# CognitiveAISystems/pogema

Measured on AMD Instinct MI355X. Metric: agent-steps/sec (whole node), 64-agent 64x64 grid, batch=8192 envs, higher is better.
Workload: dtype u32

## Files before the change

include/pogema_amd.h:

```cpp
#ifndef POGEMA_AMD_H
#define POGEMA_AMD_H

#include <stddef.h>
#include <stdint.h>

#ifdef __cplusplus
extern "C" {
#endif

#define PGX_ABI_VERSION 6

#define PGX_OK 0
#define PGX_E_INVALID (-1)
#define PGX_E_HIP (-2)
#define PGX_E_NOMEM (-3)
#define PGX_E_STATE (-4)
#define PGX_E_PLACEMENT (-5)

#define PGX_COLLISION_PRIORITY 0
#define PGX_COLLISION_BLOCK_BOTH 1
#define PGX_COLLISION_SOFT 2

#define PGX_ON_TARGET_FINISH 0
#define PGX_ON_TARGET_RESTART 1
// ... 71 lines not shown
int pgx_set_map_pool(pgx_env* env, const uint8_t* maps, int32_t num_maps, int32_t* capacity_out, void* stream);
int pgx_reset_pool(pgx_env* env, uint64_t seed, const uint8_t* env_mask, int32_t max_retries, void* stream);
int pgx_regenerate_pool(pgx_env* env, const uint8_t* env_mask, uint64_t seed, int32_t max_retries, void* obs,
                        void* stream);
int pgx_get_map_index(pgx_env* env, int32_t* map_index, void* stream);

int pgx_get_map(pgx_env* env, uint8_t* obstacles, void* stream);

int pgx_step(pgx_env* env, const void* actions, int action_dtype, void* obs, float* rewards,
             uint8_t* terminated, uint8_t* truncated, uint8_t* is_active, void* stream);

int pgx_step_held(pgx_env* env, const void* actions, int action_dtype, void* obs, uint8_t* held, int32_t refresh,
                  float* rewards, uint8_t* terminated, uint8_t* truncated, uint8_t* is_active, void* stream);
int pgx_held_available(const pgx_env* env);

int pgx_xcd_shares(pgx_env* env, int32_t* shares);
int pgx_xcd_tune(pgx_env* env, void* obs, void* obs_alt, int32_t rounds, float* us_equal, float* us_tuned, void* stream);

typedef struct pgx_geometry {
    int32_t lanes_per_env;
    int32_t waves;
    int32_t envs_per_wave;
    int32_t multi_wave;
    int32_t p16;
    int32_t stagger;
    int32_t store_policy;
    int32_t state_stores;
    int32_t grid;
    int32_t lds_bytes;
    int32_t for_rollout;
// ... 193 lines not shown
```

pogema_amd/_lib.py:

```python
from __future__ import annotations

import ctypes as C
import os

_HERE = os.path.dirname(os.path.abspath(__file__))
LIB_PATH = os.environ.get("PGX_LIB") or os.path.join(_HERE, "libpogema_amd.so")

PGX_ABI_VERSION = 6

COLLISION_SYSTEMS = {"priority": 0, "block_both": 1, "soft": 2}
ON_TARGET = {"finish": 0, "restart": 1, "nothing": 2}
ACTION_DTYPES = {"int8": 0, "int32": 1, "int64": 2}
SOFT_VERTEX_RULES = {"lowest_index": 0, "all_stay": 1}
SOFT_OCCUPANCY = {"index_order": 0, "exact": 1}
COOP_REWARDS = {"all_solved": 0, "per_agent": 1}
BAD_ACTIONS = {"noop": 0, "flag": 1}
LIFELONG_RNGS = {"build": 0, "numpy": 1}
def _obs_dtypes():
    import torch
    return {torch.float32: 0, torch.uint8: 1, torch.bfloat16: 2, torch.float16: 3}


def obs_elem_bytes(dtype) -> int:
    import torch
# ... 58 lines not shown
          "GREEDY0": TOKEN_GREEDY0, "PAD": TOKEN_PAD, "NUM_TOKENS": NUM_TOKENS, "HISTORY": TOKEN_HISTORY,
          "SLOT_LEN": TOKEN_SLOT_LEN, "MAX_SLOTS": MAX_TOKEN_SLOTS, "MAX_LENGTH": MAX_TOKEN_LENGTH}


EXPORTED_SYMBOLS = (
    "pgx_abi_version", "pgx_last_error", "pgx_create", "pgx_check_config", "pgx_destroy", "pgx_obs_elems", "pgx_agent_elems",
    "pgx_reset_from_state", "pgx_reset_random", "pgx_regenerate", "pgx_regenerate_failures", "pgx_get_map", "pgx_step", "pgx_step_held", "pgx_held_available", "pgx_observe", "pgx_set_metrics_buffers", "pgx_get_state", "pgx_generate", "pgx_place_agents",
    "pgx_snapshot_bytes", "pgx_save_snapshot", "pgx_load_snapshot", "pgx_time_observe", "pgx_bad_action_count",
    "pgx_buffers_create", "pgx_buffers_ptr", "pgx_buffers_get_info", "pgx_buffers_destroy", "pgx_set_targets",
    "pgx_np_streams", "pgx_np_streams_host", "pgx_np_generate", "pgx_np_generate_host", "pgx_rollout", "pgx_buffers_stride", "pgx_buffers_drop", "pgx_xcd_shares", "pgx_xcd_tune", "pgx_buffers_create_at", "pgx_time_observe_pair", "pgx_buffers_va_reserved", "pgx_get_geometry",
    "pgx_expert_actions", "pgx_set_map_pool", "pgx_reset_pool", "pgx_regenerate_pool", "pgx_get_map_index",
    "pgx_cost_to_go", "pgx_cost_to_go_bytes", "pgx_cost_to_go_builds", "pgx_visible_agents", "pgx_pibt_actions",
    "pgx_goal_directions", "pgx_shield_actions", "pgx_pibt_plan", "pgx_move_outcomes",
    "pgx_policy_input", "pgx_copy_envs", "pgx_global_state", "pgx_global_state_check",
    "pgx_agent_tokens", "pgx_agent_tokens_length", "pgx_goal_paths", "pgx_pibt_swap_actions",
    "pgx_agent_forecasts", "pgx_blocking",
)


class PgxError(RuntimeError):
    def __init__(self, code: int, message: str):
        super().__init__(f"pogema_amd engine error {code}: {message}")
        self.code = code


class PgxBuffersInfo(C.Structure):
    _fields_ = [("bytes", C.c_int64), ("count", C.c_int32), ("spread", C.c_int32), ("candidates", C.c_int32),
                ("reserved0", C.c_int32), ("same_zone_us", C.c_float), ("final_us", C.c_float), ("spacer_gib", C.c_double),
                ("buffer_gbs", C.c_float), ("reserved1", C.c_float)]


# ... 138 lines not shown
    lib.pgx_bad_action_count.argtypes = [vp, vp]
    lib.pgx_bad_action_count.restype = i64
    lib.pgx_time_observe.argtypes = [vp, vp, i32, C.POINTER(C.c_float), vp]
    lib.pgx_time_observe.restype = C.c_int
    lib.pgx_time_observe_pair.argtypes = [vp, vp, vp, i32, C.POINTER(C.c_float), vp]
    lib.pgx_time_observe_pair.restype = C.c_int
    lib.pgx_snapshot_bytes.argtypes = [vp]
    lib.pgx_snapshot_bytes.restype = i64
    lib.pgx_save_snapshot.argtypes = [vp, vp, vp]
    lib.pgx_load_snapshot.argtypes = [vp, vp, vp]
    lib.pgx_save_snapshot.restype = lib.pgx_load_snapshot.restype = C.c_int
    lib.pgx_step.argtypes = [vp, vp, C.c_int, vp, vp, vp, vp, vp, vp]
    lib.pgx_step_held.argtypes = [vp, vp, C.c_int, vp, vp, i32, vp, vp, vp, vp, vp]
    lib.pgx_held_available.argtypes = [vp]
    lib.pgx_step_held.restype = lib.pgx_held_available.restype = C.c_int
    lib.pgx_observe.argtypes = [vp, vp, vp]
    lib.pgx_set_metrics_buffers.argtypes = [vp, vp, vp]
    lib.pgx_get_state.argtypes = [vp, vp, vp, vp, vp, vp, vp]
    lib.pgx_generate.argtypes = [i32, i32, i32, i32, f32, u64, i64, i32, i32, vp, vp, vp]
    lib.pgx_place_agents.argtypes = [i32, i32, i32, i32, u64, i64, i32, i32, vp, i32, vp, vp]
    for name in ("pgx_create", "pgx_destroy", "pgx_reset_from_state", "pgx_reset_random", "pgx_regenerate", "pgx_get_map",
                 "pgx_step", "pgx_observe", "pgx_set_metrics_buffers", "pgx_set_metrics_buffers",
                 "pgx_get_state", "pgx_generate", "pgx_place_agents"):
        getattr(lib, name).restype = C.c_int
    if lib.pgx_abi_version() != PGX_ABI_VERSION:
        raise ImportError(f"{LIB_PATH}: ABI version {lib.pgx_abi_version()} != expected {PGX_ABI_VERSION}; rebuild")
    _lib = lib
    return lib


# ... 5 lines not shown
```

pogema_amd/buffers.py:

```python
from __future__ import annotations

import atexit
import collections
import contextlib
import ctypes as C
import os
import threading

import numpy as np
import torch

from . import _lib

_TYPESTR = {torch.float32: "<f4", torch.uint8: "|u1", torch.float16: "<f2", torch.bfloat16: "<f2"}


class _Owner:

    def __init__(self, lib, handle):
        self._lib, self._handle = lib, handle

    def __del__(self):
        try:
            if self._handle is not None and self._handle.value:
# ... 322 lines not shown
        dev = obs_tensors[0].device
        n = batch * agents
        self._sets = []
        for obs in obs_tensors:
            block = torch.empty(n * 7 + 16, dtype=torch.uint8, device=dev)
            members = (obs, block[:4 * n].view(torch.float32).view(batch, agents),
                       block[4 * n:5 * n].view(torch.bool).view(batch, agents),
                       block[5 * n:6 * n].view(torch.bool).view(batch, agents),
                       block[6 * n:7 * n].view(torch.bool).view(batch, agents))
            storages = (obs.untyped_storage(), block.untyped_storage())
            self._sets.append((members, storages, tuple(st._cdata for st in storages)))
        del obs, block, members, storages
        self._idle = [tuple(self._count(c) for c in cdata) for _, _, cdata in self._sets]
        self._held = [torch.full((batch, agents), 255, dtype=torch.uint8, device=dev) for _ in self._sets]
        self._vouched = [None] * len(self._sets)
        self._next = 0
        self.taken = 0
        self.misses = 0

    def __len__(self):
        return len(self._sets)

    def obs_pointers(self):
        return [members[0].data_ptr() for members, _, _ in self._sets]

    def _is_idle(self, i: int) -> bool:
        cdata, idle = self._sets[i][2], self._idle[i]
        return self._count(cdata[0]) == idle[0] and self._count(cdata[1]) == idle[1]

    def free_sets(self) -> int:
        return sum(self._is_idle(i) for i in range(len(self._sets)))

    def retire(self):
        idle = [i for i in range(len(self._sets)) if self._is_idle(i)]
        out = [self._sets[i][0][0] for i in idle if self._sets[i][0][0].data_ptr() in self._zone_ptrs]
        for i in reversed(idle):
            del self._sets[i]
            del self._idle[i]
            del self._held[i]
            del self._vouched[i]
        self._next = 0
        return out

    def _take_index(self):
        n = len(self._sets)
        for k in range(n):
            i = (self._next + k) % n
            if self._is_idle(i):
                self._next = (i + 1) % n
                self.taken += 1
                return i
        self.misses += 1
        return None

    def _hand_out(self, i: int, with_obs: bool):
# ... 14 lines not shown
        if with_obs:
            self._vouched[i] = None
        return self._hand_out(i, with_obs)

    def take_for_step(self, with_obs: bool = True):
        i = self._take_index()
        if i is None:
            return None
        trusted = False
        if with_obs:
            v = self._vouched[i]
            trusted = v is not None and self._version(self._sets[i][0][0]) == v
            self._vouched[i] = None
        return self._hand_out(i, with_obs), self._held[i], trusted, i

    def vouch(self, i: int):
        self._vouched[i] = self._version(self._sets[i][0][0])
```

pogema_amd/csrc/pgx_api.cpp:

```cpp
#include "../../include/pogema_amd.h"

#include <hip/hip_runtime.h>

#include <algorithm>
#include <cstdarg>
#include <cstdio>
#include <cstdlib>
#include <cstring>
#include <new>
#include <string>
#include <vector>

#include "pgx_internal.h"

namespace {
thread_local std::string g_err;
}

namespace pgx {
int fail_msg(int code, const char* fmt, ...) {
    char buf[512];
    va_list ap;
    va_start(ap, fmt);
    vsnprintf(buf, sizeof buf, fmt, ap);
// ... 350 lines not shown
        alloc(e->tcount, BA * sizeof(uint32_t));
        if (cfg->lifelong_rng == PGX_LIFELONG_RNG_NUMPY) {
            alloc(e->np_state, BA * sizeof(pgx::NpGen));
            alloc(e->np_state0, BA * sizeof(pgx::NpGen));
        }
    }
    if (err != hipSuccess) return fail_msg(alloc_code(err), "hipMalloc failed: %s", hipGetErrorString(err));
    err = hipMemset(e->regen_fail, 0, sizeof(uint32_t));
    if (err == hipSuccess) err = hipMemset(e->bad_count, 0, sizeof(uint32_t));
    if (err == hipSuccess && e->np_state0)
        err = pgx::launch_init_np_lifelong(e->np_state0, cfg->seed, cfg->env_index_base, cfg->batch, A, nullptr);
    if (err == hipSuccess && e->np_state0) err = hipStreamSynchronize(nullptr);
    if (err == hipSuccess) err = pgx::prepare_step(e->geo, e->geo_roll);
    if (err == hipSuccess && pgx::held_available(e->geo, A, e->W, obs_elem_bytes(cfg->obs_dtype)))
        err = pgx::prepare_step_held(e->geo, A, e->W);
    if (err != hipSuccess)
        return fail_msg(PGX_E_HIP, "cannot configure the step kernel (%zu bytes of LDS): %s", e->geo.lds_bytes,
                        hipGetErrorString(err));
    if (const char* spec = getenv("PGX_XCD_WEIGHTS")) {
        float f[8], sum = 0.f;
        if (sscanf(spec, "%f,%f,%f,%f,%f,%f,%f,%f", &f[0], &f[1], &f[2], &f[3], &f[4], &f[5], &f[6], &f[7]) == 8) {
            for (float q : f) sum += q > 0.f ? q : 0.f;
            if (sum > 0.f)
                for (int x = 0; x < 8; ++x) e->xcd_w[x] = (f[x] > 0.f ? f[x] : 0.f) / sum;
        }
    }
    apply_xcd_shares(e);
    err = pgx::prepare_expert(cfg->height, cfg->width);
    if (err != hipSuccess) return fail_msg(PGX_E_HIP, "cannot configure the expert kernel: %s", hipGetErrorString(err));
    if (e->flags & 4u) {
// ... 537 lines not shown
        return pgx_step(e, actions, action_dtype, obs, rewards, terminated, truncated, is_active, stream);
    if (!actions || !rewards || !terminated || !truncated) return fail_msg(PGX_E_INVALID, "pgx_step_held: null argument");
    if (const int rc = check_action_dtype("pgx_step_held", action_dtype)) return rc;
    DeviceGuard guard;
    if (const int rc = enter(guard, e, "pgx_step_held", true)) return rc;
    pgx::StepParams p = step_params(e, e->geo);
    p.mode = pgx::MODE_STEP;
    p.action_dtype = action_dtype;
    p.actions = actions;
    p.obs = static_cast<float*>(obs);
    p.rewards = rewards;
    p.terminated = terminated;
    p.truncated = truncated;
    p.act_out = is_active;
    PGX_HIP(pgx::launch_step_held(p, e->geo, held, refresh != 0, (hipStream_t)stream));
    return PGX_OK;
}

int pgx_rollout(pgx_env* e, int32_t steps, const pgx_rollout_io* io, void* stream) {
    if (!e || !io || !io->rewards || !io->terminated || !io->truncated)
        return fail_msg(PGX_E_INVALID, "pgx_rollout: null argument");
    if (io->policy_step0 < 0 || io->policy_step0 > ((int64_t)1 << 40))
        return fail_msg(PGX_E_INVALID, "pgx_rollout: policy_step0 outside 0..2^40");
    if (steps < 1) return fail_msg(PGX_E_INVALID, "pgx_rollout: steps must be >= 1, got %d", steps);
    if (const int rc = check_action_dtype("pgx_rollout", io->action_dtype)) return rc;
    if (io->obs && io->obs_slots < 1) return fail_msg(PGX_E_INVALID, "pgx_rollout: obs given but obs_slots = %d", io->obs_slots);
    DeviceGuard guard;
    if (const int rc = enter(guard, e, "pgx_rollout", true)) return rc;
    pgx::StepParams p = step_params(e, e->geo_roll);
    p.mode = pgx::MODE_STEP;
// ... 716 lines not shown
```

pogema_amd/csrc/pgx_internal.h:

```cpp
#pragma once
#include <hip/hip_runtime.h>
#include <stddef.h>
#include <stdint.h>

namespace pgx {

int fail_msg(int code, const char* fmt, ...);

#define PGX_HIP(call)                                                                                                      \
    do {                                                                                                                   \
        const hipError_t e__ = (call);                                                                                     \
        if (e__ != hipSuccess)                                                                                             \
            return pgx::fail_msg(PGX_E_HIP, "%s failed: %s (%s:%d)", #call, hipGetErrorString(e__), __FILE__, __LINE__); \
    } while (0)

struct DeviceGuard {
    int prev = -1;
    bool changed = false;
    hipError_t err = hipSuccess;
    DeviceGuard() = default;
    explicit DeviceGuard(int dev) { (void)select(dev); }
    DeviceGuard(const DeviceGuard&) = delete;
    DeviceGuard& operator=(const DeviceGuard&) = delete;
    hipError_t select(int dev) {
// ... 100 lines not shown
    const void* actions;
    float* obs;
    float* rewards;
    uint8_t* terminated;
    uint8_t* truncated;
    uint8_t* act_out;
    const uint8_t* only;
    unsigned long long* dbg;
};

struct HeldParams {
    uint8_t* held;
    int32_t refresh;
    int32_t lds_word;
    int32_t words;
};

struct RolloutParams {
    int32_t steps;
    int32_t obs_slots;
    int32_t resident_bitmap;
    int32_t reserved0;
    int64_t actions_stride;
    int64_t agents_stride;
    int64_t envs_stride;
    int64_t obs_stride;
    uint64_t policy_seed;
    int64_t policy_step0;
    int8_t* actions_out;
};
// ... 10 lines not shown
    bool big;
    bool pc;
    bool resident_bitmap;
    size_t lds_bytes;
    int grid;
    int32_t xcd_n[8], xcd_base[8];
};
StepGeometry step_geometry(int batch, int A, int bmw, int W, bool allow_p16, int epw_override, int obs_elem_bytes,
                           int waves_override, bool for_rollout = false);
hipError_t prepare_step(const StepGeometry& g, const StepGeometry& roll);
hipError_t raise_lds_limit(const void* fn, size_t lds_bytes);
hipError_t launch_step(const StepParams& p, const StepGeometry& g, hipStream_t stream);
bool held_available(const StepGeometry& g, int A, int W, int obs_elem_bytes);
hipError_t prepare_step_held(const StepGeometry& g, int A, int W);
hipError_t launch_step_held(const StepParams& p, const StepGeometry& g, uint8_t* held, bool refresh, hipStream_t stream);
int xcd_partition(int blocks, const float w[8], int32_t n[8], int32_t base[8]);
hipError_t launch_rollout(const StepParams& p, const RolloutParams& rp, const StepGeometry& g, hipStream_t stream);

hipError_t launch_pack_obstacles(const uint8_t* obstacles, const uint8_t* only, uint32_t* bm, int batch, int H, int Wd,
                                 int r, int wpr, int bmw, const OutsideParams& outside, hipStream_t stream);

struct ResetParams {
    int32_t env_begin, env_count;
    int32_t H, Wd, A, r, wpr, bmw;
    int32_t lifelong;
    int32_t given_state;
    int32_t max_retries;
    uint32_t thr;
    uint64_t gen_seed;
    int64_t env_index_base;
// ... 230 lines not shown
```

pogema_amd/csrc/pgx_kernels.hip:

```cpp
#include <hip/hip_runtime.h>
#include <stdint.h>
#include <stdlib.h>

#include <array>
#include <type_traits>
#include <map>
#include <mutex>
#include <string>
#include <vector>
#include <utility>

#include "pgx_internal.h"
#include "pgx_nprng.h"

namespace pgx {

__device__ __forceinline__ uint32_t lifelong_draw(uint64_t seed, uint64_t env_index, uint32_t agent,
                                                  uint32_t counter, uint32_t n) {
    uint64_t h = gen_sm64(seed);
    h = gen_sm64(h ^ env_index);
    h = gen_sm64(h ^ (((uint64_t)agent << 32) | counter));
    return (uint32_t)(((h >> 32) * (uint64_t)n) >> 32);
}

// ... 317 lines not shown
        }
    }
}

enum { MISC_FLAGS = 0, MISC_ARRIVED = 16, MISC_UNSOLVED = 17, MISC_OFFGOAL = 18, MISC_WORDS = 32 };

struct Carry {
    uint32_t pos = 0u, tgt = 1u;
    uint32_t ablk = 0u, anext = 0u;
    int elapsed = 0;
    int4 macc = {0, 0, 0, 0};
    bool active = false;
};
__device__ __forceinline__ uint32_t pack_action4(int a) { return (uint32_t)a <= 4u ? (uint32_t)a : 15u; }

template <int G, bool MW, bool P16, bool ROLL, bool BIG, bool PC, bool HELD, typename P, typename R, typename H = int>
__device__ __forceinline__ void step_body(P& p, R& rp, const int t, const int slot, Carry& c, [[maybe_unused]] const H& hp = H{}) {
    static_assert(!MW || G == 64, "multi-wave environments use full waves");
    static_assert(!HELD || (P16 && !ROLL && !BIG && !PC), "the held stream exists for the packed-row single-step kernels");
    static_assert(!BIG || MW, "the large-map layout runs one environment per workgroup");
    static_assert(!PC || (ROLL && !MW && P16), "the resolver / streamer pair exists for single-wave rollouts with packed rows");
    extern __shared__ __attribute__((aligned(16))) uint32_t smem[];

    const int tid = PC ? (int)(threadIdx.x & 63u) : (int)threadIdx.x;
    [[maybe_unused]] const int role = PC ? (int)(threadIdx.x >> 6) : 0;
    bool do_resolve = true;
    [[maybe_unused]] bool do_stream = true;
    if constexpr (PC) {
        do_resolve = role == 0 && t < rp.steps;
        do_stream = role == 1 && t > 0;
        if (!do_resolve && !do_stream) return;
// ... 43 lines not shown
    const int env_l = MW ? 0 : (lane / G);
    const int gbase = MW ? 0 : (lane & ~(G - 1));
    const int alane = MW ? lane : (lane & (G - 1));
    const int agent = MW ? tid : alane;
    const bool env_ok = env_l < nenv;
    const int env = env0 + env_l;
    const bool valid = env_ok && agent < A;
    const size_t gi = (size_t)env * A + agent;

    uint32_t pos = 0u, tgt = 1u;
    bool active = false;
    bool ghost_in = false;
    int act = 0, elapsed = 0;
    int4 macc = make_int4(0, 0, 0, 0);
    bool env_leader;
    [[maybe_unused]] int araw[8];
    [[maybe_unused]] bool fetch_block = false;
    if constexpr (ROLL) {
      env_leader = env_ok && agent == 0 && p.mode == MODE_STEP;
      if (do_resolve) {
        auto load_action = [&](size_t ai) -> int {
            if (p.action_dtype == 0) return ((const int8_t*)p.actions)[ai];
            if (p.action_dtype == 1) return ((const int32_t*)p.actions)[ai];
            return (int)((const int64_t*)p.actions)[ai];
        };
        const bool given = p.actions != nullptr;
        const int steps = rp.steps;
        const size_t stride = (size_t)rp.agents_stride;
        if (t == 0) {
            if (valid) {
// ... 37 lines not shown
    if (valid) {
        pos = p.pos[gi];
        tgt = p.tgt[gi];
        const uint32_t ab = p.active[gi];
        active = (ab & ACTIVE_BIT) != 0;
        ghost_in = (ab & ACTIVE_GHOST) != 0;
        if (p.mode == MODE_STEP) {
            if (p.action_dtype == 0) act = ((const int8_t*)p.actions)[gi];
            else if (p.action_dtype == 1) act = ((const int32_t*)p.actions)[gi];
            else act = (int)((const int64_t*)p.actions)[gi];
        }
    }
    if (env_ok && p.mode == MODE_STEP) elapsed = p.elapsed[env];
    env_leader = env_ok && agent == 0 && p.mode == MODE_STEP;
    if (env_leader) macc = p.macc[env];
    }

    if (do_resolve) {
        const uint32_t* g = p.obst + (size_t)env0 * bmw;
        const int n = nenv * bmw;
        const int stagger = (ROLL && t > 0) ? 0 : p.stagger;
        bool stage = true;
        if constexpr (ROLL) stage = t == 0 || !rp.resident_bitmap;
        if constexpr (BIG) stage = false;
        if (!stage) {
#pragma unroll 4
            for (int i = tid; i < n; i += NT) s_occ[i] = 0u;
        } else if (!MW && stagger > 0 && n <= 16 * 64) {
            uint32_t bmr[16];
#pragma unroll
// ... 3 lines not shown
            if (slot & 1u)
                for (int k = 0; k < stagger; ++k) __builtin_amdgcn_s_sleep(127);
#pragma unroll
            for (int k = 0; k < 16; ++k)
                if (tid + 64 * k < n) {
                    s_obst[tid + 64 * k] = bmr[k];
                    s_occ[tid + 64 * k] = 0u;
                }
        } else
#pragma unroll 4
        for (int i = tid; i < n; i += NT) {
            s_obst[i] = g[i];
            s_occ[i] = 0u;
        }
        if (MW && tid < MISC_WORDS) s_misc[tid] = 0u;
    }
    lds_sync<MW>();
    const bool dbg2 = dbg && (p.flags & 64u);
    if (dbg2 && tid == 0) p.dbg[(size_t)blk * 4 + 1] = wall_clock64();

    bool ghost = p.mode != MODE_STEP && ghost_in;
    struct StateOut {
        float rew = 0.0f;
        uint8_t term = 0;
        bool trunc = false, finished = false, do_reset = false, act = false;
        int n_arrived = 0;
    } so;
    int when_stores = p.mode == MODE_STEP ? p.state_stores : 0;
    if constexpr (PC) when_stores = 0;
    const bool late_stores = when_stores != 0;
// ... 230 lines not shown
            uint32_t b = 0u;
#pragma unroll
            for (int k = 0; k < 8; ++k) b |= pack_action4(araw[k]) << (4 * k);
            c.anext = b;
        }
      }
    }
    if (dbg && tid == 0) p.dbg[(size_t)blk * 4 + (dbg2 ? 3 : 1)] = wall_clock64();
    if (!p.obs) {
        if (late_stores) emit_state(pos, tgt, active, elapsed, macc, so);
        return;
    }
    if constexpr (PC) {
        if (!do_stream) return;
    }
    if constexpr (HELD) {
        for (int i = tid; i < hp.words; i += NT) smem[hp.lds_word + i] = 0u;
    }
    lds_sync<MW>();
    if (when_stores == 1) emit_state(pos, tgt, active, elapsed, macc, so);
    int out_slot = slot;
    if constexpr (PC) out_slot = slot == 0 ? rp.obs_slots - 1 : slot - 1;
    float* const obs_out = ROLL ? reinterpret_cast<float*>(reinterpret_cast<char*>(p.obs) + (size_t)out_slot * (size_t)rp.obs_stride) : p.obs;

    if constexpr (P16) {
        const int W_rt = W, r_rt = r;
        uint32_t* rows_base = smem;
        if constexpr (ROLL) rows_base = rp.resident_bitmap ? s_occ : smem;
        if constexpr (PC) rows_base = s_obst + epw * bmw + 2 * (epw * bmw + 2 * AS);
        auto p16_phases = [&](auto wt_tag) {
        constexpr int WT = decltype(wt_tag)::value;
        const int W = WT ? WT : W_rt;
        const int r = WT ? (WT - 1) / 2 : r_rt;
        const uint32_t wmask = (1u << W) - 1u;
        constexpr int RW = WT ? (WT + 1) / 2 : 8;
        [[maybe_unused]] uint32_t held_was = 255u;
        if constexpr (HELD) {
            if (tid < nag && !hp.refresh) held_was = hp.held[(size_t)env0 * A + tid];
        }
        uint32_t rp[3][RW];
#pragma unroll
        for (int t = 0; t < 3; ++t) {
#pragma unroll
            for (int m = 0; m < RW; ++m) rp[t][m] = 0u;
            const int item = tid + t * NT;
            if (item < nag * 3) {
                const int la = item / 3;
                const int c = item - la * 3;
                const int el = MW ? 0 : (p.a_magic ? (int)__umulhi((uint32_t)la, p.a_magic) : la);
                const uint32_t cell = s_apos[la];
                const int x = (int)(cell >> 16), y = (int)(cell & 0xFFFFu);
                if (c < 2) {
// ... 36 lines not shown
                            asm volatile("" ::: "memory");
                        }
                    }
                } else {
                    const uint32_t tc = s_atgt[la];
                    int dx = x - (int)(tc >> 16), dy = y - (int)(tc & 0xFFFFu);
                    dx = max(-r, min(r, dx));
                    dy = max(-r, min(r, dy));
                    const int hit = r - dx;
                    const uint32_t val = (1u << (r - dy)) << (16 * (hit & 1));
#pragma unroll
                    for (int m = 0; m < RW; ++m) rp[t][m] = (m == (hit >> 1)) ? val : 0u;
                }
            }
        }
        if constexpr (HELD) {
            if (tid < nag) {
                const int la = tid;
                const uint32_t cell = s_apos[la], tc = s_atgt[la];
                const int dx = max(-r, min(r, (int)(cell >> 16) - (int)(tc >> 16)));
                const int dy = max(-r, min(r, (int)(cell & 0xFFFFu) - (int)(tc & 0xFFFFu)));
                const uint32_t now = (uint32_t)((r - dx) * W + (r - dy));
                hp.held[(size_t)env0 * A + la] = (uint8_t)now;
                if (held_was < (uint32_t)(W * W)) {
                    constexpr int UL = PGX_HELD_UNIT_LOG2;
                    const uintptr_t slice = reinterpret_cast<uintptr_t>(obs_out + (size_t)env0 * A * 3 * W * W);
                    const uintptr_t plane = slice + (size_t)(la * 3 + 2) * (size_t)(W * W) * 4;
                    const uintptr_t ub = slice >> UL;
                    const int u1 = (int)(((plane + (size_t)(W * W) * 4) >> UL) - ub);
                    const int uw = (int)(((plane + held_was * 4) >> UL) - ub), un = (int)(((plane + now * 4) >> UL) - ub);
                    for (int u = (int)(((plane + ((1u << UL) - 1u)) >> UL) - ub); u < u1; ++u)
// ... 2 lines not shown
            }
        }
        lds_sync<MW>();
        uint16_t* rows16 = reinterpret_cast<uint16_t*>(rows_base);
#pragma unroll
        for (int t = 0; t < 3; ++t) {
            const int item = tid + t * NT;
            if (item < nag * 3) {
#pragma unroll
                for (int wy = 0; wy < (WT ? WT : 16); ++wy)
                    if (WT || wy < W) rows16[item * W + wy] = (uint16_t)(rp[t][wy >> 1] >> (16 * (wy & 1)));
            }
        }
        if (tid < 4) rows16[nag * 3 * W + tid] = 0;
        lds_sync<MW>();

        const int n = nag * 3 * W * W;
        const size_t base = (size_t)env0 * A * 3 * W * W;
        if constexpr (WT == 0) {
        if (p.obs_one && W >= 7) {
            uint16_t* o = reinterpret_cast<uint16_t*>(obs_out) + base;
            const int head = min(n, (int)((8 - (base & 7)) & 7));
            const int nvec = (n - head) >> 3;
            const int tail0 = head + (nvec << 3);
            if (tid < 16) {
                const int e = (tid < 8) ? tid : tail0 + (tid - 8);
                if ((tid < 8) ? (tid < head) : (e < n)) {
                    const int row = (int)__umulhi((uint32_t)e, p.w_magic);
                    o[e] = (uint16_t)((((uint32_t)rows16[row] >> (e - row * W)) & 1u) * p.obs_one);
                }
// ... 164 lines not shown
        if (p.store_policy == 0) stream32(std::integral_constant<uint32_t, 0u>{});
        else if (p.store_policy == 1) stream32(std::integral_constant<uint32_t, 1u>{});
        else stream32(std::integral_constant<uint32_t, 2u>{});
        if (when_stores == 2) emit_state(pos, tgt, active, elapsed, macc, so);
        if (dbg && !dbg2 && tid == 0) {
            __builtin_amdgcn_s_waitcnt(0);
            p.dbg[(size_t)blk * 4 + 3] = wall_clock64();
        }
    }
}

template <int G, bool MW, bool P16, bool BIG = false>
__global__ __launch_bounds__(MW ? 1024 : 64, MW ? 1 : 8) void step_kernel(const StepParams p) {
    const RolloutParams none{};
    Carry unused;
    step_body<G, MW, P16, false, BIG, false, false>(p, none, 0, 0, unused);
}

template <int G, bool MW>
__global__ __launch_bounds__(MW ? 1024 : 64, MW ? 1 : 8) void step_held(const StepParams p, const HeldParams hp) {
    const RolloutParams none{};
    Carry unused;
    step_body<G, MW, true, false, false, false, true>(p, none, 0, 0, unused, hp);
}

#ifndef PGX_ROLL_OCC
#define PGX_ROLL_OCC 4
#endif
template <int G, bool MW, bool P16, bool BIG = false, bool PC = false>
__global__ __launch_bounds__(MW ? 1024 : (PC ? 128 : 64), MW ? 1 : PGX_ROLL_OCC) void rollout_kernel(const StepParams p0, const RolloutParams rp0) {
    typedef const __attribute__((address_space(4))) char KC;
    typedef const __attribute__((address_space(4))) StepParams KP;
    typedef const __attribute__((address_space(4))) RolloutParams KR;
    static_assert(alignof(StepParams) == 8 && alignof(RolloutParams) == 8, "kernarg layout of rollout_kernel");
    constexpr size_t rp_offset = (sizeof(StepParams) + alignof(RolloutParams) - 1) / alignof(RolloutParams) * alignof(RolloutParams);
    const int steps = rp0.steps, slots = rp0.obs_slots;
    int slot = 0;
    Carry c;
// ... 333 lines not shown
    return g.lds_bytes + (size_t)held_words(slice) * 4 <= 160 * 1024;
}

hipError_t prepare_step_held(const StepGeometry& g, int A, int W) {
    const size_t slice = (size_t)g.epw * A * 3 * W * W * 4;
    return raise_lds_limit(held_fn_for(g), g.lds_bytes + (size_t)held_words(slice) * 4);
}

hipError_t launch_step_held(const StepParams& p, const StepGeometry& g, uint8_t* held, bool refresh, hipStream_t stream) {
    const void* fn = held_fn_for(g);
    if (!fn) return hipErrorInvalidValue;
    StepParams args = p;
    HeldParams h;
    const int W = 2 * p.r + 1;
    h.held = held;
    h.refresh = refresh ? 1 : 0;
    h.lds_word = (int32_t)(g.lds_bytes / 4);
    h.words = held_words((size_t)g.epw * p.num_agents * 3 * W * W * 4);
    void* kargs[] = {&args, &h};
    return hipLaunchKernel(fn, dim3(g.grid), dim3(64 * g.waves), kargs, g.lds_bytes + (size_t)h.words * 4, stream);
}

hipError_t launch_step(const StepParams& p, const StepGeometry& g, hipStream_t stream) {
    const void* fn = step_fn_for(g);
    if (!fn) return hipErrorInvalidValue;
    StepParams args = p;
    void* kargs[] = {&args};
    return hipLaunchKernel(fn, dim3(g.grid), dim3(64 * g.waves), kargs, g.lds_bytes, stream);
}


hipError_t launch_pack_obstacles(const uint8_t* obstacles, const uint8_t* only, uint32_t* bm, int batch, int H, int Wd,
                                 int r, int wpr, int bmw, const OutsideParams& outside, hipStream_t stream) {
// ... 52 lines not shown
```

pogema_amd/vec_env.py:

```python
from __future__ import annotations

import ctypes as C
import os
import warnings
from typing import Optional

import numpy as np
import torch

from . import _lib
from .grid_config import GridConfig
from .placement import PlacementMixin, choose_buffers
from .queries import QueryMixin
from .semantics import Semantics


def _as_device_index(device) -> int:
    dev = torch.device(device)
    if dev.type != "cuda":
        raise ValueError(f"VecPogema runs on a HIP device only, got {device!r}")
    return dev.index if dev.index is not None else torch.cuda.current_device()


def parse_map_pool(maps) -> torch.Tensor:
# ... 167 lines not shown
            outside_density=float(gc.density), soft_vertex_rule=_lib.SOFT_VERTEX_RULES[self.semantics.soft_vertex],
            coop_reward=_lib.COOP_REWARDS[self.semantics.coop_reward],
            bad_action=_lib.BAD_ACTIONS[self.semantics.bad_action],
            lifelong_rng=_lib.LIFELONG_RNGS[self.semantics.lifelong_rng],
            soft_occupancy=_lib.SOFT_OCCUPANCY[self.semantics.soft_occupancy], abi_version=_lib.PGX_ABI_VERSION)
        self._handle = C.c_void_p()
        rc = self._lib.pgx_check_config(C.byref(cfg))
        if rc != 0:
            raise ValueError(f"this GridConfig does not fit the engine: {self._lib.pgx_last_error().decode()} (README.md, Limits)")
        _lib.check(self._lib.pgx_create(C.byref(cfg), self.device_index, C.byref(self._handle)))
        if held_zeros is None and os.environ.get("PGX_HELD_ZEROS") in ("0", "1"):
            held_zeros = os.environ["PGX_HELD_ZEROS"] == "1"
        self._held_on = ((self._held_pays() if held_zeros is None else bool(held_zeros)) and self.recycle
                         and self.obs_dtype == torch.float32 and not self.regenerate
                         and bool(self._lib.pgx_held_available(self._handle)))
        self._held_steps = 0
        self._held_refreshes = 0
        self._bufs = None
        self._buf_i = 0
        self._shared = None
        self._reset_seed = None
        self._initial = None
        self._pool = None
        self.metrics = torch.zeros((self.batch, len(_lib.METRIC_NAMES)), dtype=torch.float32, device=self.device)
        self.episode_done = torch.zeros((self.batch,), dtype=torch.bool, device=self.device)
        _lib.check(self._lib.pgx_set_metrics_buffers(self._handle, self.metrics.data_ptr(), self.episode_done.data_ptr()))
        if pool is not None:
            self.set_map_pool(pool)

    def close(self, release: bool = False):
# ... 317 lines not shown
        self.placement = dict(placement or {}, adopted=True)
        if self.placement_probe and self.batch >= 2048 and self._has_state():
            self.placement.update(self.tune_xcd_shares(tensors[0], tensors[-1] if len(tensors) > 1 else None))
        return self.placement

    def _has_state(self):
        return self._initial is not None

    HELD_MIN_BYTES = 128 << 20

    def _held_pays(self) -> bool:
        return int(np.prod(self.obs_shape)) * 4 >= self.HELD_MIN_BYTES

    @property
    def held_zeros(self) -> dict:
        return {"enabled": bool(self._held_on), "steps": self._held_steps, "refreshes": self._held_refreshes}

    def _outputs(self, with_obs: bool = True):
        if self.recycle:
            return self._recycled(with_obs)
        if not self.reuse_buffers:
            return self._alloc_outputs(with_obs)
        if self._bufs is None:
            if torch.cuda.is_current_stream_capturing():
                raise RuntimeError("reuse_buffers: the output buffers are picked by a timed zone walk that synchronises "
                                   "the device -- call warm_buffers() (or one un-captured step) before capturing")
            self.warm_buffers()
        self._buf_i = 0 if self.single_buffer else self._buf_i ^ 1
        return self._bufs[self._buf_i]

    def observe(self, out: Optional[torch.Tensor] = None) -> torch.Tensor:
# ... 34 lines not shown
            if tuple(t.shape) != tuple(shape) or not ok_dtype or not t.is_contiguous() or t.device != self.device:
                raise ValueError(f"out[{name}] must be a contiguous {dtype} tensor of shape {tuple(shape)} on {self.device}")
        return out

    def step(self, actions, compute_obs: bool = True, out=None):
        actions = self._prepare_actions(actions)
        if out is not None:
            obs, rewards, terminated, truncated, is_active = self._check_out(out)
            if compute_obs and obs is None:
                raise ValueError("out[obs] is None but compute_obs=True")
        else:
            held = self._held_outputs(compute_obs) if self._held_on else None
            if held is not None:
                (obs, rewards, terminated, truncated, is_active), record, trusted, index = held
                if compute_obs:
                    _lib.check(self._lib.pgx_step_held(
                        self._handle, actions.data_ptr(), self._ACTION_CODE[actions.dtype], obs.data_ptr(), record.data_ptr(),
                        0 if trusted else 1, rewards.data_ptr(), terminated.data_ptr(), truncated.data_ptr(),
                        is_active.data_ptr(), self._stream()))
                    self._recycler.vouch(index)
                    self._held_steps += 1
                    self._held_refreshes += 0 if trusted else 1
                    infos = {"is_active": is_active, "episode_done": self.episode_done, "metrics": self.metrics}
                    if self.semantics.bad_action == "flag":
                        self._raise_on_bad_actions()
                    return self._wrap_obs(obs), rewards, terminated, truncated, infos
            elif self._held_on and self._recycler and not torch.cuda.is_current_stream_capturing():
                obs, rewards, terminated, truncated, is_active = self._alloc_outputs(compute_obs)
            else:
                obs, rewards, terminated, truncated, is_active = self._outputs(compute_obs)
        _lib.check(self._lib.pgx_step(
# ... 178 lines not shown
```

Baseline: 5.344 billion.

## Add line-granular held-zero record to skip rewriting all-zero observation units

Adds a new held-stream step kernel variant that records, per 128-byte unit of each env slice's observation output, whether the unit was all zeros on the previous write into a recycled buffer. The kernel ORs packed row bits per unit, ballots the zero flags into a per-block bitmask kept in LDS and global memory, and uses it to skip stores of units that are already zero in the reused buffer. The aim is to cut global write bandwidth for float32 observations, replacing the per-agent target-based held rule. It costs extra LDS, a ballot pass and a record buffer per recycled set, and is picked by default only for large observations when the multi-wave helper layout does not apply.

```diff
diff --git a/include/pogema_amd.h b/include/pogema_amd.h
--- a/include/pogema_amd.h
+++ b/include/pogema_amd.h
@@ -109,6 +109,10 @@
                   float* rewards, uint8_t* terminated, uint8_t* truncated, uint8_t* is_active, void* stream);
 int pgx_held_available(const pgx_env* env);
 
+int pgx_step_held_lines(pgx_env* env, const void* actions, int action_dtype, void* obs, uint32_t* lines, int32_t refresh,
+                        float* rewards, uint8_t* terminated, uint8_t* truncated, uint8_t* is_active, void* stream);
+int64_t pgx_held_lines_words(const pgx_env* env);
+
 int pgx_xcd_shares(pgx_env* env, int32_t* shares);
 int pgx_xcd_tune(pgx_env* env, void* obs, void* obs_alt, int32_t rounds, float* us_equal, float* us_tuned, void* stream);
 
diff --git a/pogema_amd/_lib.py b/pogema_amd/_lib.py
--- a/pogema_amd/_lib.py
+++ b/pogema_amd/_lib.py
@@ -96,7 +96,7 @@
     "pgx_goal_directions", "pgx_shield_actions", "pgx_pibt_plan", "pgx_move_outcomes",
     "pgx_policy_input", "pgx_copy_envs", "pgx_global_state", "pgx_global_state_check",
     "pgx_agent_tokens", "pgx_agent_tokens_length", "pgx_goal_paths", "pgx_pibt_swap_actions",
-    "pgx_agent_forecasts", "pgx_blocking",
+    "pgx_agent_forecasts", "pgx_blocking", "pgx_step_held_lines", "pgx_held_lines_words",
 )
 
 
@@ -265,6 +265,10 @@
     lib.pgx_step_held.argtypes = [vp, vp, C.c_int, vp, vp, i32, vp, vp, vp, vp, vp]
     lib.pgx_held_available.argtypes = [vp]
     lib.pgx_step_held.restype = lib.pgx_held_available.restype = C.c_int
+    lib.pgx_step_held_lines.argtypes = [vp, vp, C.c_int, vp, vp, i32, vp, vp, vp, vp, vp]
+    lib.pgx_step_held_lines.restype = C.c_int
+    lib.pgx_held_lines_words.argtypes = [vp]
+    lib.pgx_held_lines_words.restype = i64
     lib.pgx_observe.argtypes = [vp, vp, vp]
     lib.pgx_set_metrics_buffers.argtypes = [vp, vp, vp]
     lib.pgx_get_state.argtypes = [vp, vp, vp, vp, vp, vp, vp]
diff --git a/pogema_amd/buffers.py b/pogema_amd/buffers.py
--- a/pogema_amd/buffers.py
+++ b/pogema_amd/buffers.py
@@ -360,6 +360,7 @@
         self._idle = [tuple(self._count(c) for c in cdata) for _, _, cdata in self._sets]
         self._held = [torch.full((batch, agents), 255, dtype=torch.uint8, device=dev) for _ in self._sets]
         self._vouched = [None] * len(self._sets)
+        self._lines = [None] * len(self._sets)
         self._next = 0
         self.taken = 0
         self.misses = 0
@@ -385,6 +386,7 @@
             del self._idle[i]
             del self._held[i]
             del self._vouched[i]
+            del self._lines[i]
         self._next = 0
         return out
 
@@ -429,5 +431,11 @@
             self._vouched[i] = None
         return self._hand_out(i, with_obs), self._held[i], trusted, i
 
+    def line_record(self, i: int, words: int):
+        rec = self._lines[i]
+        if rec is None or rec.numel() != words:
+            rec = self._lines[i] = torch.zeros(words, dtype=torch.int32, device=self._sets[i][0][0].device)
+        return rec
+
     def vouch(self, i: int):
         self._vouched[i] = self._version(self._sets[i][0][0])
diff --git a/pogema_amd/csrc/pgx_api.cpp b/pogema_amd/csrc/pgx_api.cpp
--- a/pogema_amd/csrc/pgx_api.cpp
+++ b/pogema_amd/csrc/pgx_api.cpp
@@ -388,6 +388,8 @@
     if (err == hipSuccess) err = pgx::prepare_step(e->geo, e->geo_roll);
     if (err == hipSuccess && pgx::held_available(e->geo, A, e->W, obs_elem_bytes(cfg->obs_dtype)))
         err = pgx::prepare_step_held(e->geo, A, e->W);
+    if (err == hipSuccess && pgx::held_lines_words(e->geo, cfg->batch, A, e->W, obs_elem_bytes(cfg->obs_dtype)))
+        err = pgx::prepare_step_held_lines(e->geo, A, e->W);
     if (err != hipSuccess)
         return fail_msg(PGX_E_HIP, "cannot configure the step kernel (%zu bytes of LDS): %s", e->geo.lds_bytes,
                         hipGetErrorString(err));
@@ -955,6 +957,32 @@
     p.truncated = truncated;
     p.act_out = is_active;
     PGX_HIP(pgx::launch_step_held(p, e->geo, held, refresh != 0, (hipStream_t)stream));
+    return PGX_OK;
+}
+
+int64_t pgx_held_lines_words(const pgx_env* e) {
+    if (!e) return 0;
+    return pgx::held_lines_words(e->geo, e->cfg.batch, e->cfg.num_agents, e->W, obs_elem_bytes(e->cfg.obs_dtype));
+}
+
+int pgx_step_held_lines(pgx_env* e, const void* actions, int action_dtype, void* obs, uint32_t* lines, int32_t refresh,
+                        float* rewards, uint8_t* terminated, uint8_t* truncated, uint8_t* is_active, void* stream) {
+    if (!e || !obs || !lines || !pgx_held_lines_words(e))
+        return pgx_step(e, actions, action_dtype, obs, rewards, terminated, truncated, is_active, stream);
+    if (!actions || !rewards || !terminated || !truncated) return fail_msg(PGX_E_INVALID, "pgx_step_held_lines: null argument");
+    if (const int rc = check_action_dtype("pgx_step_held_lines", action_dtype)) return rc;
+    DeviceGuard guard;
+    if (const int rc = enter(guard, e, "pgx_step_held_lines", true)) return rc;
+    pgx::StepParams p = step_params(e, e->geo);
+    p.mode = pgx::MODE_STEP;
+    p.action_dtype = action_dtype;
+    p.actions = actions;
+    p.obs = static_cast<float*>(obs);
+    p.rewards = rewards;
+    p.terminated = terminated;
+    p.truncated = truncated;
+    p.act_out = is_active;
+    PGX_HIP(pgx::launch_step_held_lines(p, e->geo, lines, refresh != 0, (hipStream_t)stream));
     return PGX_OK;
 }
 
diff --git a/pogema_amd/csrc/pgx_internal.h b/pogema_amd/csrc/pgx_internal.h
--- a/pogema_amd/csrc/pgx_internal.h
+++ b/pogema_amd/csrc/pgx_internal.h
@@ -138,6 +138,7 @@
     int32_t refresh;
     int32_t lds_word;
     int32_t words;
+    uint32_t* lines;
 };
 
 struct RolloutParams {
@@ -178,6 +179,9 @@
 bool held_available(const StepGeometry& g, int A, int W, int obs_elem_bytes);
 hipError_t prepare_step_held(const StepGeometry& g, int A, int W);
 hipError_t launch_step_held(const StepParams& p, const StepGeometry& g, uint8_t* held, bool refresh, hipStream_t stream);
+long held_lines_words(const StepGeometry& g, int batch, int A, int W, int obs_elem_bytes);
+hipError_t prepare_step_held_lines(const StepGeometry& g, int A, int W);
+hipError_t launch_step_held_lines(const StepParams& p, const StepGeometry& g, uint32_t* lines, bool refresh, hipStream_t stream);
 int xcd_partition(int blocks, const float w[8], int32_t n[8], int32_t base[8]);
 hipError_t launch_rollout(const StepParams& p, const RolloutParams& rp, const StepGeometry& g, hipStream_t stream);
 
diff --git a/pogema_amd/csrc/pgx_kernels.hip b/pogema_amd/csrc/pgx_kernels.hip
--- a/pogema_amd/csrc/pgx_kernels.hip
+++ b/pogema_amd/csrc/pgx_kernels.hip
@@ -355,7 +355,7 @@
 };
 __device__ __forceinline__ uint32_t pack_action4(int a) { return (uint32_t)a <= 4u ? (uint32_t)a : 15u; }
 
-template <int G, bool MW, bool P16, bool ROLL, bool BIG, bool PC, bool HELD, typename P, typename R, typename H = int>
+template <int G, bool MW, bool P16, bool ROLL, bool BIG, bool PC, int HELD, typename P, typename R, typename H = int>
 __device__ __forceinline__ void step_body(P& p, R& rp, const int t, const int slot, Carry& c, [[maybe_unused]] const H& hp = H{}) {
     static_assert(!MW || G == 64, "multi-wave environments use full waves");
     static_assert(!HELD || (P16 && !ROLL && !BIG && !PC), "the held stream exists for the packed-row single-step kernels");
@@ -429,6 +429,7 @@
     int act = 0, elapsed = 0;
     int4 macc = make_int4(0, 0, 0, 0);
     bool env_leader;
+    [[maybe_unused]] uint32_t lines_old = 0u;
     [[maybe_unused]] int araw[8];
     [[maybe_unused]] bool fetch_block = false;
     if constexpr (ROLL) {
@@ -496,6 +497,9 @@
     if (env_ok && p.mode == MODE_STEP) elapsed = p.elapsed[env];
     env_leader = env_ok && agent == 0 && p.mode == MODE_STEP;
     if (env_leader) macc = p.macc[env];
+    if constexpr (HELD == 2) {
+        if (tid < hp.words && !hp.refresh) lines_old = hp.lines[(size_t)blk * hp.words + tid];
+    }
     }
 
     if (do_resolve) {
@@ -529,6 +533,9 @@
             s_occ[i] = 0u;
         }
         if (MW && tid < MISC_WORDS) s_misc[tid] = 0u;
+    }
+    if constexpr (HELD == 2) {
+        if (tid < hp.words) smem[hp.lds_word + tid] = lines_old;
     }
     lds_sync<MW>();
     const bool dbg2 = dbg && (p.flags & 64u);
@@ -789,7 +796,7 @@
     if constexpr (PC) {
         if (!do_stream) return;
     }
-    if constexpr (HELD) {
+    if constexpr (HELD == 1) {
         for (int i = tid; i < hp.words; i += NT) smem[hp.lds_word + i] = 0u;
     }
     lds_sync<MW>();
@@ -810,7 +817,7 @@
         const uint32_t wmask = (1u << W) - 1u;
         constexpr int RW = WT ? (WT + 1) / 2 : 8;
         [[maybe_unused]] uint32_t held_was = 255u;
-        if constexpr (HELD) {
+        if constexpr (HELD == 1) {
             if (tid < nag && !hp.refresh) held_was = hp.held[(size_t)env0 * A + tid];
         }
         uint32_t rp[3][RW];
@@ -877,7 +884,7 @@
                 }
             }
         }
-        if constexpr (HELD) {
+        if constexpr (HELD == 1) {
             if (tid < nag) {
                 const int la = tid;
                 const uint32_t cell = s_apos[la], tc = s_atgt[la];
@@ -910,6 +917,40 @@
         }
         if (tid < 4) rows16[nag * 3 * W + tid] = 0;
         lds_sync<MW>();
+        if constexpr (HELD == 2) {
+            constexpr int UL = PGX_HELD_UNIT_LOG2;
+            static_assert(UL == 7, "one lane ORs the 32 float cells of a 128-byte unit");
+            constexpr int KR = WT ? (30 + 2 * WT) / WT : 1;
+            [[maybe_unused]] const int kr = (30 + 2 * W) / W;
+            const int n = nag * 3 * W * W, nrows = nag * 3 * W;
+            const uintptr_t slice = reinterpret_cast<uintptr_t>(obs_out + (size_t)env0 * A * 3 * W * W);
+            const int lead = (int)((slice & ((1u << UL) - 1u)) >> 2);
+            for (int u0 = wave << 6; u0 < (hp.words << 5); u0 += NT) {
+                const int f0 = ((u0 + lane) << 5) - lead;
+                const bool inside = f0 >= 0 && f0 + 32 <= n;
+                const int w = (u0 >> 5) + (lane >> 5);
+                const bool writer = (lane & 31) == 0 && w < hp.words;
+                uint32_t oldw = 0u;
+                if (writer) oldw = smem[hp.lds_word + w];
+                const int row = (int)__umulhi((uint32_t)(inside ? f0 : 0), p.w_magic);
+                const int col = (inside ? f0 : 0) - row * W;
+                uint64_t cells = 0u;
+                if constexpr (WT != 0) {
+#pragma unroll
+                    for (int k = 0; k < KR; ++k) cells |= (uint64_t)rows16[min(row + k, nrows)] << (k * W);
+                } else {
+#pragma nounroll
+                    for (int k = 0; k < kr; ++k) cells |= (uint64_t)rows16[min(row + k, nrows)] << (k * W);
+                }
+                const uint64_t zero = __ballot(inside && (uint32_t)(cells >> col) == 0u);
+                if (writer) {
+                    const uint32_t z = (uint32_t)(zero >> lane);
+                    smem[hp.lds_word + w] = oldw & z;
+                    hp.lines[(size_t)blk * hp.words + w] = z;
+                }
+            }
+            lds_sync<MW>();
+        }
 
         const int n = nag * 3 * W * W;
         const size_t base = (size_t)env0 * A * 3 * W * W;
@@ -1104,14 +1145,21 @@
 __global__ __launch_bounds__(MW ? 1024 : 64, MW ? 1 : 8) void step_kernel(const StepParams p) {
     const RolloutParams none{};
     Carry unused;
-    step_body<G, MW, P16, false, BIG, false, false>(p, none, 0, 0, unused);
+    step_body<G, MW, P16, false, BIG, false, 0>(p, none, 0, 0, unused);
 }
 
 template <int G, bool MW>
 __global__ __launch_bounds__(MW ? 1024 : 64, MW ? 1 : 8) void step_held(const StepParams p, const HeldParams hp) {
     const RolloutParams none{};
     Carry unused;
-    step_body<G, MW, true, false, false, false, true>(p, none, 0, 0, unused, hp);
+    step_body<G, MW, true, false, false, false, 1>(p, none, 0, 0, unused, hp);
+}
+
+template <int G, bool MW>
+__global__ __launch_bounds__(MW ? 1024 : 64, MW ? 1 : 8) void step_held_lines(const StepParams p, const HeldParams hp) {
+    const RolloutParams none{};
+    Carry unused;
+    step_body<G, MW, true, false, false, false, 2>(p, none, 0, 0, unused, hp);
 }
 
 #ifndef PGX_ROLL_OCC
@@ -1475,9 +1523,50 @@
     HeldParams h;
     const int W = 2 * p.r + 1;
     h.held = held;
+    h.lines = nullptr;
     h.refresh = refresh ? 1 : 0;
     h.lds_word = (int32_t)(g.lds_bytes / 4);
     h.words = held_words((size_t)g.epw * p.num_agents * 3 * W * W * 4);
+    void* kargs[] = {&args, &h};
+    return hipLaunchKernel(fn, dim3(g.grid), dim3(64 * g.waves), kargs, g.lds_bytes + (size_t)h.words * 4, stream);
+}
+
+static const void* held_lines_fn_for(const StepGeometry& g) {
+    if (g.big || !g.p16) return nullptr;
+    if (g.multi_wave) return reinterpret_cast<const void*>(&step_held_lines<64, true>);
+#define PGX_CASE(gg) case gg: return reinterpret_cast<const void*>(&step_held_lines<gg, false>);
+    switch (g.G) {
+        PGX_CASE(1) PGX_CASE(2) PGX_CASE(4) PGX_CASE(8) PGX_CASE(16) PGX_CASE(32) PGX_CASE(64)
+        default: return nullptr;
+    }
+#undef PGX_CASE
+}
+
+static long held_slices(const StepGeometry& g, int batch) { return g.multi_wave ? batch : (batch + g.epw - 1) / g.epw; }
+
+long held_lines_words(const StepGeometry& g, int batch, int A, int W, int obs_elem_bytes) {
+    if (!held_lines_fn_for(g) || !held_available(g, A, W, obs_elem_bytes)) return 0;
+    const int words = held_words((size_t)g.epw * A * 3 * W * W * 4);
+    if (words > 64 * g.waves) return 0;
+    return held_slices(g, batch) * words;
+}
+
+hipError_t prepare_step_held_lines(const StepGeometry& g, int A, int W) {
+    const size_t slice = (size_t)g.epw * A * 3 * W * W * 4;
+    return raise_lds_limit(held_lines_fn_for(g), g.lds_bytes + (size_t)held_words(slice) * 4);
+}
+
+hipError_t launch_step_held_lines(const StepParams& p, const StepGeometry& g, uint32_t* lines, bool refresh, hipStream_t stream) {
+    const void* fn = held_lines_fn_for(g);
+    if (!fn) return hipErrorInvalidValue;
+    StepParams args = p;
+    HeldParams h;
+    const int W = 2 * p.r + 1;
+    h.held = nullptr;
+    h.refresh = refresh ? 1 : 0;
+    h.lds_word = (int32_t)(g.lds_bytes / 4);
+    h.words = held_words((size_t)g.epw * p.num_agents * 3 * W * W * 4);
+    h.lines = lines;
     void* kargs[] = {&args, &h};
     return hipLaunchKernel(fn, dim3(g.grid), dim3(64 * g.waves), kargs, g.lds_bytes + (size_t)h.words * 4, stream);
 }
diff --git a/pogema_amd/vec_env.py b/pogema_amd/vec_env.py
--- a/pogema_amd/vec_env.py
+++ b/pogema_amd/vec_env.py
@@ -205,6 +205,12 @@
         self._held_on = ((self._held_pays() if held_zeros is None else bool(held_zeros)) and self.recycle
                          and self.obs_dtype == torch.float32 and not self.regenerate
                          and bool(self._lib.pgx_held_available(self._handle)))
+        self._held_line_words = int(self._lib.pgx_held_lines_words(self._handle)) if self._held_on else 0
+        helpers = self.num_agents <= 64 and bool(self.geometry()["multi_wave"])
+        rule = os.environ.get("PGX_HELD_RULE") or ("lines" if self._held_pays() and not helpers else "target")
+        if rule not in ("target", "lines"):
+            raise ValueError(f"PGX_HELD_RULE must be 'target' or 'lines', got {rule!r}")
+        self._held_rule = rule if self._held_line_words > 0 else "target"
         self._held_steps = 0
         self._held_refreshes = 0
         self._bufs = None
@@ -552,7 +558,8 @@
 
     @property
     def held_zeros(self) -> dict:
-        return {"enabled": bool(self._held_on), "steps": self._held_steps, "refreshes": self._held_refreshes}
+        return {"enabled": bool(self._held_on), "steps": self._held_steps, "refreshes": self._held_refreshes,
+                "rule": self._held_rule}
 
     def _outputs(self, with_obs: bool = True):
         if self.recycle:
@@ -617,7 +624,12 @@
             if held is not None:
                 (obs, rewards, terminated, truncated, is_active), record, trusted, index = held
                 if compute_obs:
-                    _lib.check(self._lib.pgx_step_held(
+                    if self._held_rule == "lines":
+                        record = self._recycler.line_record(index, self._held_line_words)
+                        held_step = self._lib.pgx_step_held_lines
+                    else:
+                        held_step = self._lib.pgx_step_held
+                    _lib.check(held_step(
                         self._handle, actions.data_ptr(), self._ACTION_CODE[actions.dtype], obs.data_ptr(), record.data_ptr(),
                         0 if trusted else 1, rewards.data_ptr(), terminated.data_ptr(), truncated.data_ptr(),
                         is_active.data_ptr(), self._stream()))
```

After: 4.515 billion. 0.845x the previous value.
